# irlyngaas/UCF-VIT

Hardware: AMD Instinct MI355X
Metric: images/sec/node ViT-L/16 224^2 bf16 train step (higher is better)
Workload: dtype bf16; 1 GPU; vit_l16_224 train step (fwd+bwd+AdamW), synthetic U{0..255} images resident in HBM; per_gpu_batch=665, global_batch=665, parallelism=dp1, grad_all_reduce=none (1 rank)

## Files before the change

### ucf-vit_amd/csrc/attention_short.hip

```cpp
#include "attn_route.h"
#include "attn_tile.h"

namespace {

constexpr int AS_THREADS = 256;

template <typename T, int DH, int NB> struct AS {
    static constexpr int EPV = 16 / sizeof(T);
    static constexpr int RB = DH * sizeof(T);
    static constexpr int SPR = RB / 16;
    static constexpr int NCH = DH / (4 * EPV);
    static constexpr int NDB = DH / 16;
    static constexpr int BPC = (4 * EPV) / 16;
    static constexpr int NRC = (NB + BPC - 1) / BPC;
    static constexpr int ROWS = NRC * BPC * 16;
    static constexpr int IMG = ROWS * RB;
    typedef typename Mma16<T>::frag_t frag_t;
};

template <typename T, int DH, int ROWS>
__device__ __forceinline__ void load_image(char* lds, const T* __restrict__ base, int64_t row_stride, int R, int tid) {
    constexpr int EPV = 16 / sizeof(T), SPR = DH * sizeof(T) / 16;
    constexpr int NIT = (ROWS * SPR + AS_THREADS - 1) / AS_THREADS;
    u32x4 v[NIT];
#pragma unroll
    for (int i = 0; i < NIT; ++i) {
        const int p = tid + i * AS_THREADS;
        const int row = p / SPR, slot = p % SPR;
        v[i] = u32x4{0u, 0u, 0u, 0u};
        if (p < ROWS * SPR && row < R) v[i] = *reinterpret_cast<const u32x4*>(base + (int64_t)row * row_stride + slot * EPV);
    }
#pragma unroll
    for (int i = 0; i < NIT; ++i) {
        const int p = tid + i * AS_THREADS;
        if (p < ROWS * SPR) *reinterpret_cast<u32x4*>(lds + tile_off<T, DH>(p / SPR, p % SPR)) = v[i];
    }
}

template <typename T, int DH, int NB, bool EXACT>
__global__ __launch_bounds__(AS_THREADS) void attn_s_fwd_kernel(const T* __restrict__ qkv, T* __restrict__ out, float* __restrict__ lse, int N,
                                                                 int H, float scale_log2e) {
    typedef AS<T, DH, NB> A;
    typedef typename A::frag_t frag_t;
    extern __shared__ __attribute__((aligned(16))) char smem[];
    char* ldsK = smem;
    char* ldsV = smem + A::IMG;
    const int tid = threadIdx.x, lane = tid & 63, wave = tid >> 6, g = lane >> 4, li = lane & 15;
    const int h = blockIdx.x % H;
    const int64_t b = blockIdx.x / H;
    const int D = H * DH;
    const int64_t rs = 3 * (int64_t)D;
    const T* qbase = qkv + b * N * rs + h * DH;
    load_image<T, DH, A::ROWS>(ldsK, qbase + D, rs, N, tid);
    load_image<T, DH, A::ROWS>(ldsV, qbase + 2 * D, rs, N, tid);
    __syncthreads();
    const int nqb = (N + 15) / 16;
    for (int qb = wave; qb < nqb; qb += 4) {
        const int q = qb * 16 + li;
        frag_t qf[A::NCH];
#pragma unroll
        for (int c = 0; c < A::NCH; ++c) qf[c] = frag_global<T, DH>(qbase, rs, q, N, c, lane);
        f32x4 s[NB];
        float mx = -INFINITY;
#pragma unroll
        for (int kb = 0; kb < NB; ++kb) {
            s[kb] = f32x4{0.f, 0.f, 0.f, 0.f};
#pragma unroll
            for (int c = 0; c < A::NCH; ++c) Mma16<T>::mma(s[kb], frag_row<T, DH>(ldsK, kb, c, lane), qf[c]);
            if (EXACT ? (kb == NB - 1) : (kb * 16 + 16 > N)) {
#pragma unroll
                for (int r = 0; r < 4; ++r) s[kb][r] = (kb * 16 + 4 * g + r < N) ? s[kb][r] : -INFINITY;
            }
#pragma unroll
            for (int r = 0; r < 4; ++r) mx = fmaxf(mx, s[kb][r]);
        }
        const float m = group_max(mx) * scale_log2e;
        float l = 0.f;
#pragma unroll
        for (int kb = 0; kb < NB; ++kb)
#pragma unroll
            for (int r = 0; r < 4; ++r) {
                const float p = __builtin_amdgcn_exp2f(fmaf(s[kb][r], scale_log2e, -m));
                s[kb][r] = p;
                l += p;
            }
        const float lt = group_sum(l);
        f32x4 o[A::NDB];
#pragma unroll
        for (int d = 0; d < A::NDB; ++d) o[d] = f32x4{0.f, 0.f, 0.f, 0.f};
#pragma unroll
        for (int rc = 0; rc < A::NRC; ++rc) {
            const frag_t pf = frag_from_acc<T, NB>(s, rc);
#pragma unroll
            for (int d = 0; d < A::NDB; ++d) Mma16<T>::mma(o[d], frag_tr<T, DH>(ldsV, rc, d, lane), pf);
        }
        if (q < N) {
            const float inv = 1.f / lt;
            T* op = out + (b * N + q) * D + h * DH;
#pragma unroll
            for (int d = 0; d < A::NDB; ++d) {
                Vec4<T> v;
#pragma unroll
                for (int r = 0; r < 4; ++r) v.set(r, o[d][r] * inv);
                *reinterpret_cast<Vec4<T>*>(op + d * 16 + 4 * g) = v;
            }
            if (g == 0) lse[(b * H + h) * N + q] = m + log2f(lt);
        }
    }
}

template <int RB> __device__ __forceinline__ bf16x8 af_row(const char* img, int base_c, int blk) {
    return *reinterpret_cast<const bf16x8*>(img + base_c + blk * (16 * RB));
}
template <int RB> __device__ __forceinline__ bf16x8 af_tr(const char* img, int base_d, int rc) {
    const char* a = img + base_d + rc * (32 * RB);
    short4v lo = __builtin_amdgcn_ds_read_tr16_b64_v4i16(LDS_PTR(short4v, a));
    short4v hi = __builtin_amdgcn_ds_read_tr16_b64_v4i16(LDS_PTR(short4v, a + 16 * RB));
    short8v r = {lo[0], lo[1], lo[2], lo[3], hi[0], hi[1], hi[2], hi[3]};
    return __builtin_bit_cast(bf16x8, r);
}
template <int DH> struct AfBases {
    int rowb[DH / 32], trb;
    __device__ __forceinline__ AfBases(int lane) {
        constexpr int RB = DH * 2, SPR = RB / 16;
        const int g = lane >> 4, li = lane & 15, tq = li >> 2, tp = li & 3;
        const int sw_row = slot_swz<SPR>(li);
#pragma unroll
        for (int c = 0; c < DH / 32; ++c) rowb[c] = li * RB + (((4 * c + g) ^ sw_row) << 4);
        const int sw_tr = slot_swz<SPR>(4 * g + tq);
        trb = (4 * g + tq) * RB + ((((tp >> 1) ^ sw_tr)) << 4) + (tp & 1) * 8;
    }
};

constexpr int AG_THREADS = 256, AG_WAVES = 4;

template <int ROWS, int DH> struct AgStage {
    static constexpr int SPR = DH / 8;
    static constexpr int NIT = (ROWS * SPR + AG_THREADS - 1) / AG_THREADS;
    u32x4 v[NIT];
};
template <int ROWS, int DH>
__device__ __forceinline__ void ag_fetch(AgStage<ROWS, DH>& st, const bf16* __restrict__ base, int64_t row_stride, int R, int tid) {
    constexpr int SPR = DH / 8;
#pragma unroll
    for (int i = 0; i < AgStage<ROWS, DH>::NIT; ++i) {
        const int p = tid + i * AG_THREADS;
        const int row = p / SPR, slot = p % SPR;
        st.v[i] = u32x4{0u, 0u, 0u, 0u};
        if (p < ROWS * SPR && row < R) st.v[i] = *reinterpret_cast<const u32x4*>(base + (int64_t)row * row_stride + slot * 8);
    }
}
template <int ROWS, int DH>
__device__ __forceinline__ void ag_fetch(AgStage<ROWS, DH>& st, __amdgpu_buffer_rsrc_t r, int byte0, int row_bytes, int tid) {
    constexpr int SPR = DH / 8;
#pragma unroll
    for (int i = 0; i < AgStage<ROWS, DH>::NIT; ++i) {
        const int p = tid + i * AG_THREADS;
        st.v[i] = __builtin_amdgcn_raw_buffer_load_b128(r, byte0 + (p / SPR) * row_bytes + (p % SPR) * 16, 0, 0);
    }
}
template <int ROWS, int DH> __device__ __forceinline__ void ag_store(const AgStage<ROWS, DH>& st, char* lds, int tid) {
    constexpr int SPR = DH / 8;
#pragma unroll
    for (int i = 0; i < AgStage<ROWS, DH>::NIT; ++i) {
        const int p = tid + i * AG_THREADS;
        if (p < ROWS * SPR) *reinterpret_cast<u32x4*>(lds + tile_off<bf16, DH>(p / SPR, p % SPR)) = st.v[i];
    }
}

__device__ __forceinline__ bf16x8 ag_pack(const f32x4& lo, const f32x4& hi) {
    bf16x8 r;
#pragma unroll
    for (int j = 0; j < 4; ++j) {
        r[j] = (bf16)lo[j];
        r[4 + j] = (bf16)hi[j];
    }
    return r;
}

#ifdef AG_STAMP
__device__ unsigned long long g_ag_stamps[4][32];
#define AG_STAMP_HERE(k)                                                                                        \
    do {                                                                                                        \
        if (blockIdx.x == gridDim.x / 2 && (threadIdx.x & 63) == 0) g_ag_stamps[threadIdx.x >> 6][k] = __builtin_amdgcn_s_memtime(); \
    } while (0)
#else
#define AG_STAMP_HERE(k) do { } while (0)
#endif

template <int DH, int NB, bool EXACT> struct AgCtx {
    static constexpr int RB = DH * 2, NCH = DH / 32, NDB = DH / 16, NRC = (NB + 1) / 2;
    const char *slot0, *slot1;
    const float *ldsLse, *ldsDelta;
    int rowb[NCH], trb, N, g, li, lane;
    float scale, sl2;
};

template <int NJ, int NCH> struct AgOpsA {
    bf16x8 qf[NJ][NCH], dof[NJ][NCH], of[NJ][NCH];
};
template <int NJ, int NCH> struct AgOpsB {
    bf16x8 kf[NJ][NCH], vf[NJ][NCH];
};

template <int DH> __device__ __forceinline__ bf16x8 ag_frag(__amdgpu_buffer_rsrc_t r, int byte0, int row, int row_bytes, int c, int lane) {
    return __builtin_bit_cast(bf16x8, __builtin_amdgcn_raw_buffer_load_b128(r, byte0 + row * row_bytes + (4 * c + (lane >> 4)) * 16, 0, 0));
}
template <int NJ, int DH>
__device__ __forceinline__ void ag_a_fetch(AgOpsA<NJ, DH / 32>& o, int blk0, __amdgpu_buffer_rsrc_t rQ, int rs_bytes, __amdgpu_buffer_rsrc_t rDO,
                                           __amdgpu_buffer_rsrc_t rO, int d_bytes, int li, int lane) {
#pragma unroll
    for (int j = 0; j < NJ; ++j) {
        const int q = (blk0 + j) * 16 + li;
#pragma unroll
        for (int c = 0; c < DH / 32; ++c) {
            o.qf[j][c] = ag_frag<DH>(rQ, 0, q, rs_bytes, c, lane);
            o.dof[j][c] = ag_frag<DH>(rDO, 0, q, d_bytes, c, lane);
            o.of[j][c] = ag_frag<DH>(rO, 0, q, d_bytes, c, lane);
        }
    }
}
template <int NJ, int DH>
__device__ __forceinline__ void ag_b_fetch(AgOpsB<NJ, DH / 32>& o, int blk0, __amdgpu_buffer_rsrc_t rQ, int rs_bytes, int d_bytes, int li, int lane) {
#pragma unroll
    for (int j = 0; j < NJ; ++j) {
        const int key = (blk0 + j) * 16 + li;
#pragma unroll
        for (int c = 0; c < DH / 32; ++c) {
            o.kf[j][c] = ag_frag<DH>(rQ, d_bytes, key, rs_bytes, c, lane);
            o.vf[j][c] = ag_frag<DH>(rQ, 2 * d_bytes, key, rs_bytes, c, lane);
        }
    }
}
__device__ __forceinline__ void ag_store4(__amdgpu_buffer_rsrc_t r, int byte_off, const f32x4& v, float mul) {
    Vec4<bf16> o;
#pragma unroll
    for (int i = 0; i < 4; ++i) o.set(i, v[i] * mul);
    __builtin_amdgcn_raw_buffer_store_b64(__builtin_bit_cast(u32x2, o), r, byte_off, 0, 0);
}

__device__ __forceinline__ float ag_row16_sum(float t) {
#define AG_DPP(x, ctrl) __builtin_bit_cast(float, __builtin_amdgcn_update_dpp(0, __builtin_bit_cast(int, x), ctrl, 0xF, 0xF, true))
    t += AG_DPP(t, 0xB1);
    t += AG_DPP(t, 0x4E);
    t += AG_DPP(t, 0x141);
    t += AG_DPP(t, 0x140);
#undef AG_DPP
    return t;
}

template <int NDB> __device__ __forceinline__ void ag_colsum_add(float (&v)[NDB][4], float* __restrict__ row, int g, int li, float mul) {
#pragma unroll
    for (int d = 0; d < NDB; ++d)
#pragma unroll
        for (int r = 0; r < 4; ++r) {
            const float t = ag_row16_sum(v[d][r]);
            if (li == 0) row[d * 16 + 4 * g + r] += t * mul;
        }
}

template <int NJ, int DH, int NB, bool EXACT>
__device__ __forceinline__ void ag_dq_pass(const AgCtx<DH, NB, EXACT>& cx, int blk0, const AgOpsA<NJ, DH / 32>& o, float* __restrict__ ldsDeltaW,
                                           __amdgpu_buffer_rsrc_t rDQ, int rs_bytes, float* __restrict__ cs_row) {
    typedef bf16 T;
    typedef AgCtx<DH, NB, EXACT> C;
    constexpr int RB = C::RB, NCH = C::NCH, NDB = C::NDB, NRC = C::NRC;
    const int N = cx.N, g = cx.g, li = cx.li;
    float neg_lse[NJ], neg_delta[NJ];
#pragma unroll
    for (int j = 0; j < NJ; ++j) {
        const int q = (blk0 + j) * 16 + li;
        float dl = 0.f;
#pragma unroll
        for (int c = 0; c < NCH; ++c)
#pragma unroll
            for (int i = 0; i < 8; ++i) dl = fmaf((float)o.dof[j][c][i], (float)o.of[j][c][i], dl);
        neg_delta[j] = -group_sum(dl);
        neg_lse[j] = -cx.ldsLse[q];
        if (g == 0) ldsDeltaW[q] = neg_delta[j];
    }
    f32x4 dq[NJ][NDB];
#pragma unroll
    for (int j = 0; j < NJ; ++j)
#pragma unroll
        for (int d = 0; d < NDB; ++d) dq[j][d] = f32x4{0.f, 0.f, 0.f, 0.f};
#pragma unroll
    for (int rc = 0; rc < NRC; ++rc) {
        f32x4 dst[NJ][2];
#pragma unroll
        for (int h2 = 0; h2 < 2; ++h2) {
            const int kb = 2 * rc + h2;
            if (kb < NB) {
                bf16x8 kfr[NCH], vfr[NCH];
#pragma unroll
                for (int c = 0; c < NCH; ++c) {
                    kfr[c] = af_row<RB>(cx.slot0, cx.rowb[c], kb);
                    vfr[c] = af_row<RB>(cx.slot1, cx.rowb[c], kb);
                }
#pragma unroll
                for (int j = 0; j < NJ; ++j) {
                    f32x4 sacc = {0.f, 0.f, 0.f, 0.f}, dp = {neg_delta[j], neg_delta[j], neg_delta[j], neg_delta[j]};
#pragma unroll
                    for (int c = 0; c < NCH; ++c) {
                        Mma16<T>::mma(sacc, kfr[c], o.qf[j][c]);
                        Mma16<T>::mma(dp, vfr[c], o.dof[j][c]);
                    }
#pragma unroll
                    for (int r = 0; r < 4; ++r) {
                        float p = __builtin_amdgcn_exp2f(fmaf(sacc[r], cx.sl2, neg_lse[j]));
                        if (EXACT ? (kb == NB - 1) : (kb * 16 + 16 > N)) p = (kb * 16 + 4 * g + r < N) ? p : 0.f;
                        dst[j][h2][r] = p * dp[r];
                    }
                }
            } else {
#pragma unroll
                for (int j = 0; j < NJ; ++j) dst[j][h2] = f32x4{0.f, 0.f, 0.f, 0.f};
            }
        }
        bf16x8 f[NJ];
#pragma unroll
        for (int j = 0; j < NJ; ++j) f[j] = ag_pack(dst[j][0], dst[j][1]);
#pragma unroll
        for (int d = 0; d < NDB; ++d) {
            const bf16x8 ktr = af_tr<RB>(cx.slot0, cx.trb ^ (d << 5), rc);
#pragma unroll
            for (int j = 0; j < NJ; ++j) Mma16<T>::mma(dq[j][d], ktr, f[j]);
        }
        __builtin_amdgcn_sched_barrier(0);
#ifdef AG_STAMP
        if (blk0 < AG_WAVES * NJ) AG_STAMP_HERE(17 + rc);
        else AG_STAMP_HERE(24 + rc);
#endif
    }
#pragma unroll
    for (int j = 0; j < NJ; ++j) {
        const int q = (blk0 + j) * 16 + li;
#pragma unroll
        for (int d = 0; d < NDB; ++d) ag_store4(rDQ, q * rs_bytes + d * 32 + 8 * g, dq[j][d], cx.scale);
    }
    if (cs_row) {
        float v[NDB][4];
#pragma unroll
        for (int d = 0; d < NDB; ++d)
#pragma unroll
            for (int r = 0; r < 4; ++r) {
                v[d][r] = dq[0][d][r];
#pragma unroll
                for (int j = 1; j < NJ; ++j) v[d][r] += dq[j][d][r];
            }
        ag_colsum_add<NDB>(v, cs_row, g, li, cx.scale);
    }
}

template <int NJ, int DH, int NB, bool EXACT>
__device__ __forceinline__ void ag_dkv_pass(const AgCtx<DH, NB, EXACT>& cx, int blk0, const AgOpsB<NJ, DH / 32>& o, __amdgpu_buffer_rsrc_t rDQ, int rs_bytes,
                                            int d_bytes) {
    typedef bf16 T;
    typedef AgCtx<DH, NB, EXACT> C;
    constexpr int RB = C::RB, NCH = C::NCH, NDB = C::NDB, NRC = C::NRC;
    const int N = cx.N, g = cx.g, li = cx.li;
    f32x4 dk[NJ][NDB], dv[NJ][NDB];
#pragma unroll
    for (int j = 0; j < NJ; ++j)
#pragma unroll
        for (int d = 0; d < NDB; ++d) {
            dk[j][d] = f32x4{0.f, 0.f, 0.f, 0.f};
            dv[j][d] = f32x4{0.f, 0.f, 0.f, 0.f};
        }
#pragma unroll
    for (int rc = 0; rc < NRC; ++rc) {
        f32x4 pt[NJ][2], st[NJ][2];
#pragma unroll
        for (int h2 = 0; h2 < 2; ++h2) {
            const int qb = 2 * rc + h2;
            if (qb < NB) {
                bf16x8 qfr[NCH], dofr[NCH];
#pragma unroll
                for (int c = 0; c < NCH; ++c) {
                    qfr[c] = af_row<RB>(cx.slot0, cx.rowb[c], qb);
                    dofr[c] = af_row<RB>(cx.slot1, cx.rowb[c], qb);
                }
                const f32x4 l4 = *reinterpret_cast<const f32x4*>(cx.ldsLse + qb * 16 + 4 * g);
                const f32x4 nd4 = *reinterpret_cast<const f32x4*>(cx.ldsDelta + qb * 16 + 4 * g);
#pragma unroll
                for (int j = 0; j < NJ; ++j) {
                    f32x4 sacc = {0.f, 0.f, 0.f, 0.f}, dp = nd4;
#pragma unroll
                    for (int c = 0; c < NCH; ++c) {
                        Mma16<T>::mma(sacc, qfr[c], o.kf[j][c]);
                        Mma16<T>::mma(dp, dofr[c], o.vf[j][c]);
                    }
#pragma unroll
                    for (int r = 0; r < 4; ++r) {
                        const float p = __builtin_amdgcn_exp2f(fmaf(sacc[r], cx.sl2, -l4[r]));
                        pt[j][h2][r] = p;
                        st[j][h2][r] = p * dp[r];
                    }
                }
            } else {
#pragma unroll
                for (int j = 0; j < NJ; ++j) {
                    pt[j][h2] = f32x4{0.f, 0.f, 0.f, 0.f};
                    st[j][h2] = f32x4{0.f, 0.f, 0.f, 0.f};
                }
            }
        }
        bf16x8 fp[NJ], fs[NJ];
#pragma unroll
        for (int j = 0; j < NJ; ++j) {
            fp[j] = ag_pack(pt[j][0], pt[j][1]);
            fs[j] = ag_pack(st[j][0], st[j][1]);
        }
#pragma unroll
        for (int d = 0; d < NDB; ++d) {
            const bf16x8 dotr = af_tr<RB>(cx.slot1, cx.trb ^ (d << 5), rc);
            const bf16x8 qtr = af_tr<RB>(cx.slot0, cx.trb ^ (d << 5), rc);
#pragma unroll
            for (int j = 0; j < NJ; ++j) {
                Mma16<T>::mma(dv[j][d], dotr, fp[j]);
                Mma16<T>::mma(dk[j][d], qtr, fs[j]);
            }
        }
        __builtin_amdgcn_sched_barrier(0);
    }
#pragma unroll
    for (int j = 0; j < NJ; ++j) {
        const int key = (blk0 + j) * 16 + li;
#pragma unroll
        for (int d = 0; d < NDB; ++d) {
            ag_store4(rDQ, d_bytes + key * rs_bytes + d * 32 + 8 * g, dk[j][d], cx.scale);
            ag_store4(rDQ, 2 * d_bytes + key * rs_bytes + d * 32 + 8 * g, dv[j][d], 1.f);
        }
    }
}

template <int DH, int NB, bool EXACT>
__global__ __launch_bounds__(AG_THREADS, 2) void attn_g_bwd_kernel(const bf16* __restrict__ qkv, const bf16* __restrict__ out,
                                                                 const bf16* __restrict__ dout, const float* __restrict__ lse,
                                                                 bf16* __restrict__ dqkv, float* __restrict__ cs_partial, int N, int H, float scale,
                                                                 float scale_log2e) {
    typedef bf16 T;
    constexpr int RB = DH * 2, NCH = DH / 32, NRC = (NB + 1) / 2, ROWS = NRC * 32, IMG = ROWS * RB, NJ = NB > 8 ? 2 : 1;
    extern __shared__ __attribute__((aligned(16))) char smem[];
    char* slot0 = smem;
    char* slot1 = smem + IMG;
    float* ldsLse = reinterpret_cast<float*>(smem + 2 * IMG);
    float* ldsDelta = ldsLse + ROWS;
    float* ldsCs = ldsDelta + ROWS;
    const int tid = threadIdx.x, lane = tid & 63, li = lane & 15;
    const int wave = __builtin_amdgcn_readfirstlane(tid >> 6);
    const int h = blockIdx.x % H;
    const int64_t b = blockIdx.x / H;
    const int D = H * DH;
    const int64_t rs = 3 * (int64_t)D;
    const T* qbase = qkv + b * N * rs + h * DH;
    const T* dobase = dout + b * N * (int64_t)D + h * DH;
    const T* obase = out + b * N * (int64_t)D + h * DH;
    T* dqbase = dqkv + b * N * rs + h * DH;
    const float* lse_bh = lse + (b * H + h) * N;
    const int nqb = (N + 15) / 16;
    constexpr int STEP = AG_WAVES * NJ;
    const int rs_bytes = (int)rs * 2, d_bytes = D * 2;
    const __amdgpu_buffer_rsrc_t rQ = buffer_rsrc(qbase, N * rs_bytes), rDO = buffer_rsrc(dobase, N * d_bytes), rO = buffer_rsrc(obase, N * d_bytes),
                                 rDQ = buffer_rsrc(dqbase, N * rs_bytes);
    AG_STAMP_HERE(0);
    AgOpsA<NJ, NCH> oa, oa2;
    ag_a_fetch<NJ, DH>(oa, wave * NJ, rQ, rs_bytes, rDO, rO, d_bytes, li, lane);
    {
        AgStage<ROWS, DH> sk, sv;
        ag_fetch<ROWS, DH>(sk, rQ, d_bytes, rs_bytes, tid);
        ag_fetch<ROWS, DH>(sv, rQ, 2 * d_bytes, rs_bytes, tid);
        ag_store<ROWS, DH>(sk, slot0, tid);
        ag_store<ROWS, DH>(sv, slot1, tid);
    }
    AG_STAMP_HERE(1);
    for (int i = tid; i < ROWS; i += AG_THREADS) {
        ldsLse[i] = i < N ? lse_bh[i] : INFINITY;
        ldsDelta[i] = 0.f;
    }
    if (cs_partial)
        for (int i = tid; i < AG_WAVES * DH; i += AG_THREADS) ldsCs[i] = 0.f;
    float* cs_row = cs_partial ? ldsCs + wave * DH : nullptr;
    AgStage<ROWS, DH> sq, sdo;
    ag_fetch<ROWS, DH>(sq, rQ, 0, rs_bytes, tid);
    ag_fetch<ROWS, DH>(sdo, rDO, 0, d_bytes, tid);
    ag_a_fetch<NJ, DH>(oa2, wave * NJ + STEP, rQ, rs_bytes, rDO, rO, d_bytes, li, lane);
    __syncthreads();
    AG_STAMP_HERE(2);

    const AfBases<DH> ab(lane);
    AgCtx<DH, NB, EXACT> cx;
    cx.slot0 = slot0;
    cx.slot1 = slot1;
    cx.ldsLse = ldsLse;
    cx.ldsDelta = ldsDelta;
#pragma unroll
    for (int c = 0; c < NCH; ++c) cx.rowb[c] = ab.rowb[c];
    cx.trb = ab.trb;
    cx.N = N;
    cx.g = lane >> 4;
    cx.li = li;
    cx.lane = lane;
    cx.scale = scale;
    cx.sl2 = scale_log2e;

    ag_dq_pass<NJ>(cx, wave * NJ, oa, ldsDelta, rDQ, rs_bytes, cs_row);
    AG_STAMP_HERE(3);
    if (wave * NJ + STEP < nqb) ag_dq_pass<NJ>(cx, wave * NJ + STEP, oa2, ldsDelta, rDQ, rs_bytes, cs_row);
    AG_STAMP_HERE(4);
    const int bw = AG_WAVES - 1 - wave;
    AgOpsB<NJ, NCH> ob, ob2;
#pragma unroll
    for (int j = 0; j < NJ; ++j)
#pragma unroll
        for (int c = 0; c < NCH; ++c) {
            ob.kf[j][c] = *reinterpret_cast<const bf16x8*>(slot0 + cx.rowb[c] + (bw * NJ + j) * (16 * RB));
            ob.vf[j][c] = *reinterpret_cast<const bf16x8*>(slot1 + cx.rowb[c] + (bw * NJ + j) * (16 * RB));
        }
    AG_STAMP_HERE(8);
    __syncthreads();
    AG_STAMP_HERE(9);
    ag_store<ROWS, DH>(sq, slot0, tid);
    ag_store<ROWS, DH>(sdo, slot1, tid);
    ag_b_fetch<NJ, DH>(ob2, bw * NJ + STEP, rQ, rs_bytes, d_bytes, li, lane);
    __syncthreads();
    AG_STAMP_HERE(10);

    ag_dkv_pass<NJ>(cx, bw * NJ, ob, rDQ, rs_bytes, d_bytes);
    AG_STAMP_HERE(11);
    if (bw * NJ + STEP < nqb) ag_dkv_pass<NJ>(cx, bw * NJ + STEP, ob2, rDQ, rs_bytes, d_bytes);
    AG_STAMP_HERE(16);
    if (cs_partial) {
        for (int i = tid; i < 2 * DH; i += AG_THREADS) {
            const int d = i % DH;
            const float t = (ldsCs[d] + ldsCs[DH + d]) + (ldsCs[2 * DH + d] + ldsCs[3 * DH + d]);
            cs_partial[b * (2 * D) + (i / DH) * D + h * DH + d] = i < DH ? t : 0.f;
        }
    }
}


template <int DH, int NB, bool EXACT>
__global__ __launch_bounds__(AG_THREADS, 3) void attn_s3_fwd_kernel(const bf16* __restrict__ qkv, bf16* __restrict__ out, float* __restrict__ lse,
                                                                     int N, int H, float scale_log2e) {
    typedef bf16 T;
    constexpr int RB = DH * 2, NCH = DH / 32, NDB = DH / 16, NRC = (NB + 1) / 2, ROWS = NB * 16, IMG = ROWS * RB;
    static_assert(NRC * 32 - ROWS <= 16, "the last transposed chunk may only run into K's first 16 rows");
    extern __shared__ __attribute__((aligned(16))) char smem[];
    char* ldsV = smem;
    char* ldsK = smem + IMG;
    const int tid = threadIdx.x, lane = tid & 63, g = lane >> 4, li = lane & 15;
    const int wave = __builtin_amdgcn_readfirstlane(tid >> 6);
    const int h = blockIdx.x % H;
    const int64_t b = blockIdx.x / H;
    const int D = H * DH;
    const int64_t rs = 3 * (int64_t)D;
    const T* qbase = qkv + b * N * rs + h * DH;
    constexpr int NPASS = (NB + AG_WAVES - 1) / AG_WAVES;
    const int rs_bytes = (int)rs * 2;
    const __amdgpu_buffer_rsrc_t rQ = buffer_rsrc(qbase, N * rs_bytes);
    bf16x8 qf_all[NPASS][NCH];
#pragma unroll
    for (int i = 0; i < NPASS; ++i)
#pragma unroll
        for (int c = 0; c < NCH; ++c) qf_all[i][c] = ag_frag<DH>(rQ, 0, (wave + i * AG_WAVES) * 16 + li, rs_bytes, c, lane);
    {
        AgStage<ROWS, DH> sk, sv;
        ag_fetch<ROWS, DH>(sk, rQ, D * 2, rs_bytes, tid);
        ag_fetch<ROWS, DH>(sv, rQ, 2 * D * 2, rs_bytes, tid);
        ag_store<ROWS, DH>(sk, ldsK, tid);
        ag_store<ROWS, DH>(sv, ldsV, tid);
    }
    __syncthreads();
    const AfBases<DH> ab(lane);
    const int trb = ab.trb;
    const int nqb = (N + 15) / 16;
#pragma unroll
    for (int ps = 0; ps < NPASS; ++ps) {
        const int qb = wave + ps * AG_WAVES;
        if (qb >= nqb) break;
        const int q = qb * 16 + li;
        bf16x8 qf[NCH];
#pragma unroll
        for (int c = 0; c < NCH; ++c) qf[c] = qf_all[ps][c];
        f32x4 s[NB];
        float mx = -INFINITY;
#pragma unroll
        for (int kb = 0; kb < NB; ++kb) {
            s[kb] = f32x4{0.f, 0.f, 0.f, 0.f};
#pragma unroll
            for (int c = 0; c < NCH; ++c) Mma16<T>::mma(s[kb], af_row<RB>(ldsK, ab.rowb[c], kb), qf[c]);
            if (EXACT ? (kb == NB - 1) : (kb * 16 + 16 > N)) {
#pragma unroll
                for (int r = 0; r < 4; ++r) s[kb][r] = (kb * 16 + 4 * g + r < N) ? s[kb][r] : -INFINITY;
            }
#pragma unroll
            for (int r = 0; r < 4; ++r) mx = fmaxf(mx, s[kb][r]);
            if ((kb & 3) == 3) __builtin_amdgcn_sched_barrier(0);
        }
        const float m = group_max(mx) * scale_log2e;
        float l = 0.f;
#pragma unroll
        for (int kb = 0; kb < NB; ++kb)
#pragma unroll
            for (int r = 0; r < 4; ++r) {
                const float p = __builtin_amdgcn_exp2f(fmaf(s[kb][r], scale_log2e, -m));
                s[kb][r] = p;
                l += p;
            }
        const float lt = group_sum(l);
        f32x4 o[NDB];
#pragma unroll
        for (int d = 0; d < NDB; ++d) o[d] = f32x4{0.f, 0.f, 0.f, 0.f};
#pragma unroll
        for (int rc = 0; rc < NRC; ++rc) {
            const bf16x8 pf = frag_from_acc<T, NB>(s, rc);
#pragma unroll
            for (int d = 0; d < NDB; ++d) Mma16<T>::mma(o[d], af_tr<RB>(ldsV, trb ^ (d << 5), rc), pf);
            __builtin_amdgcn_sched_barrier(0);
        }
        if (q < N) {
            const float inv = 1.f / lt;
            T* op = out + (b * N + q) * D + h * DH;
#pragma unroll
            for (int d = 0; d < NDB; ++d) {
                Vec4<T> v;
#pragma unroll
                for (int r = 0; r < 4; ++r) v.set(r, o[d][r] * inv);
                *reinterpret_cast<Vec4<T>*>(op + d * 16 + 4 * g) = v;
            }
            if (g == 0) lse[(b * H + h) * N + q] = m + log2f(lt);
        }
    }
}


static_assert(AS_THREADS == AG_THREADS, "one block size for the three families");

struct ShortFwd {
    static constexpr const char* name = "ucfvit_attention_fwd(short)";
    static constexpr bool has(int nb) { return nb != 13; }
    template <int DH, int NB> static constexpr size_t smem() { return 2 * AS<bf16, DH, NB>::IMG; }
    template <int DH, int NB, bool EXACT> static auto kernel() { return attn_s_fwd_kernel<bf16, DH, NB, EXACT>; }
};
struct S3Fwd {
    static constexpr const char* name = "ucfvit_attention_fwd(short, 3 per CU)";
    static constexpr bool has(int nb) { return nb == 13; }
    template <int DH, int NB> static constexpr size_t smem() { return 2 * (size_t)NB * 16 * (DH * 2); }
    template <int DH, int NB, bool EXACT> static auto kernel() { return attn_s3_fwd_kernel<DH, NB, EXACT>; }
};
struct FusedBwd {
    static constexpr const char* name = "ucfvit_attention_bwd(fused)";
    static constexpr bool has(int nb) { return true; }
    template <int DH, int NB> static constexpr size_t smem() {
        constexpr int ROWS = ((NB + 1) / 2) * 32;
        return 2 * (size_t)ROWS * (DH * 2) + 2 * ROWS * sizeof(float) + AG_WAVES * DH * sizeof(float);
    }
    template <int DH, int NB, bool EXACT> static auto kernel() { return attn_g_bwd_kernel<DH, NB, EXACT>; }
};

template <class F, int DH, int NB, bool EXACT, typename... A> int launch_inst(int64_t BH, hipStream_t s, A... args) {
    if constexpr (F::has(NB)) {
        constexpr size_t smem = F::template smem<DH, NB>();
        const auto kern = F::template kernel<DH, NB, EXACT>();
        if (int rc = raise_lds_limit(kern, smem, "attention(short)")) return rc;
        hipLaunchKernelGGL(kern, dim3((unsigned)BH), dim3(AS_THREADS), smem, s, args...);
        UCF_LAUNCH_CHECK(F::name);
        return UCFVIT_OK;
    } else {
        ucfvit_set_error("%s: no kernel for %d blocks", F::name, NB);
        return UCFVIT_ERR_HIP;
    }
}
template <class F, int DH, int NB, typename... A> int pick_exact(const AttnRoute& r, int64_t BH, hipStream_t s, A... args) {
    return r.exact ? launch_inst<F, DH, NB, true>(BH, s, args...) : launch_inst<F, DH, NB, false>(BH, s, args...);
}
template <class F, int DH, typename... A> int pick_nb(const AttnRoute& r, int64_t BH, hipStream_t s, A... args) {
    switch (r.nb) {
        case 4: return pick_exact<F, DH, 4>(r, BH, s, args...);
        case 8: return pick_exact<F, DH, 8>(r, BH, s, args...);
        case 13: return pick_exact<F, DH, 13>(r, BH, s, args...);
        default: return pick_exact<F, DH, 16>(r, BH, s, args...);
    }
}
template <class F, typename... A> int launch_short(const AttnRoute& r, int64_t dh, int64_t BH, hipStream_t s, A... args) {
    return dh == 64 ? pick_nb<F, 64>(r, BH, s, args...) : pick_nb<F, 32>(r, BH, s, args...);
}

}

#ifdef AG_STAMP
extern "C" int ucfvit_debug_attn_stamps(unsigned long long* out) {
    return (int)hipMemcpyFromSymbol(out, HIP_SYMBOL(g_ag_stamps), sizeof(unsigned long long) * 4 * 32);
}
#endif

int ucfvit_attn_launch_short_fwd(const AttnRoute& r, const void* qkv, void* out, float* lse, int64_t B, int64_t N, int64_t H, int64_t dh,
                                 float scale, void* stream) {
    const hipStream_t s = (hipStream_t)stream;
    const float sl2 = scale * LOG2E_F;
    if (r.family == AK_S3_FWD) return launch_short<S3Fwd>(r, dh, B * H, s, (const bf16*)qkv, (bf16*)out, lse, (int)N, (int)H, sl2);
    return launch_short<ShortFwd>(r, dh, B * H, s, (const bf16*)qkv, (bf16*)out, lse, (int)N, (int)H, sl2);
}

int ucfvit_attn_launch_fused_bwd(const AttnRoute& r, const void* qkv, const void* out, const void* dout, const float* lse, void* dqkv,
                                 float* cs_partial, int64_t B, int64_t N, int64_t H, int64_t dh, float scale, void* stream) {
    return launch_short<FusedBwd>(r, dh, B * H, (hipStream_t)stream, (const bf16*)qkv, (const bf16*)out, (const bf16*)dout, lse, (bf16*)dqkv,
                                  cs_partial, (int)N, (int)H, scale, scale * LOG2E_F);
}
```

Before: 2709 images/sec.

## Reuse register-resident Q/dO and LDS K/V fragments instead of refetching from global

The attention backward kernel no longer stages Q and dO from global memory a second time for the dK/dV pass. Instead, the Q/dO fragments each wave already holds in registers are written into LDS, and the second K/V block set is read from LDS rather than through buffer loads. This removes redundant global traffic and staging registers. It adds bounds-guarded LDS writes whose correctness depends on fragment layout matching the image layout, and it may change register pressure.

```diff
diff --git a/ucf-vit_amd/csrc/attention_short.hip b/ucf-vit_amd/csrc/attention_short.hip
--- a/ucf-vit_amd/csrc/attention_short.hip
+++ b/ucf-vit_amd/csrc/attention_short.hip
@@ -220,15 +220,42 @@
         }
     }
 }
-template <int NJ, int DH>
-__device__ __forceinline__ void ag_b_fetch(AgOpsB<NJ, DH / 32>& o, int blk0, __amdgpu_buffer_rsrc_t rQ, int rs_bytes, int d_bytes, int li, int lane) {
+template <int NJ, int DH, int NBLK, int BASE>
+__device__ __forceinline__ void ag_b_take(AgOpsB<NJ, DH / 32>& o, int w, const char* imgK, const char* imgV, const int (&rowb)[DH / 32]) {
+    constexpr int RB = DH * 2;
 #pragma unroll
     for (int j = 0; j < NJ; ++j) {
-        const int key = (blk0 + j) * 16 + li;
+        const int blk = BASE + w * NJ + j;
 #pragma unroll
         for (int c = 0; c < DH / 32; ++c) {
-            o.kf[j][c] = ag_frag<DH>(rQ, d_bytes, key, rs_bytes, c, lane);
-            o.vf[j][c] = ag_frag<DH>(rQ, 2 * d_bytes, key, rs_bytes, c, lane);
+            o.kf[j][c] = bf16x8{};
+            o.vf[j][c] = bf16x8{};
+        }
+        if (BASE + j < NBLK) {
+            if (BASE + (AG_WAVES - 1) * NJ + j < NBLK || blk < NBLK) {
+#pragma unroll
+                for (int c = 0; c < DH / 32; ++c) {
+                    o.kf[j][c] = af_row<RB>(imgK, rowb[c], blk);
+                    o.vf[j][c] = af_row<RB>(imgV, rowb[c], blk);
+                }
+            }
+        }
+    }
+}
+template <int NJ, int DH, int NBLK, int BASE>
+__device__ __forceinline__ void ag_a_put(const AgOpsA<NJ, DH / 32>& o, int w, char* imgQ, char* imgDO, const int (&rowb)[DH / 32]) {
+    constexpr int RB = DH * 2;
+#pragma unroll
+    for (int j = 0; j < NJ; ++j) {
+        const int blk = BASE + w * NJ + j;
+        if (BASE + j < NBLK) {
+            if (BASE + (AG_WAVES - 1) * NJ + j < NBLK || blk < NBLK) {
+#pragma unroll
+                for (int c = 0; c < DH / 32; ++c) {
+                    *reinterpret_cast<bf16x8*>(imgQ + rowb[c] + blk * (16 * RB)) = o.qf[j][c];
+                    *reinterpret_cast<bf16x8*>(imgDO + rowb[c] + blk * (16 * RB)) = o.dof[j][c];
+                }
+            }
         }
     }
 }
@@ -481,9 +508,6 @@
     if (cs_partial)
         for (int i = tid; i < AG_WAVES * DH; i += AG_THREADS) ldsCs[i] = 0.f;
     float* cs_row = cs_partial ? ldsCs + wave * DH : nullptr;
-    AgStage<ROWS, DH> sq, sdo;
-    ag_fetch<ROWS, DH>(sq, rQ, 0, rs_bytes, tid);
-    ag_fetch<ROWS, DH>(sdo, rDO, 0, d_bytes, tid);
     ag_a_fetch<NJ, DH>(oa2, wave * NJ + STEP, rQ, rs_bytes, rDO, rO, d_bytes, li, lane);
     __syncthreads();
     AG_STAMP_HERE(2);
@@ -510,19 +534,13 @@
     AG_STAMP_HERE(4);
     const int bw = AG_WAVES - 1 - wave;
     AgOpsB<NJ, NCH> ob, ob2;
-#pragma unroll
-    for (int j = 0; j < NJ; ++j)
-#pragma unroll
-        for (int c = 0; c < NCH; ++c) {
-            ob.kf[j][c] = *reinterpret_cast<const bf16x8*>(slot0 + cx.rowb[c] + (bw * NJ + j) * (16 * RB));
-            ob.vf[j][c] = *reinterpret_cast<const bf16x8*>(slot1 + cx.rowb[c] + (bw * NJ + j) * (16 * RB));
-        }
+    ag_b_take<NJ, DH, ROWS / 16, 0>(ob, bw, slot0, slot1, cx.rowb);
+    ag_b_take<NJ, DH, ROWS / 16, STEP>(ob2, bw, slot0, slot1, cx.rowb);
     AG_STAMP_HERE(8);
     __syncthreads();
     AG_STAMP_HERE(9);
-    ag_store<ROWS, DH>(sq, slot0, tid);
-    ag_store<ROWS, DH>(sdo, slot1, tid);
-    ag_b_fetch<NJ, DH>(ob2, bw * NJ + STEP, rQ, rs_bytes, d_bytes, li, lane);
+    ag_a_put<NJ, DH, ROWS / 16, 0>(oa, wave, slot0, slot1, cx.rowb);
+    ag_a_put<NJ, DH, ROWS / 16, STEP>(oa2, wave, slot0, slot1, cx.rowb);
     __syncthreads();
     AG_STAMP_HERE(10);
 
```

Measured after the change: 2715 images/sec (median of 6 runs). Within noise of the previous version (+0.2%).
